# libmir/mir-optim

Hardware: AMD Instinct MI355X
Metric: LM iterations/sec (higher is better)
Workload: dtype f64

## Files before the change

mir_optim_amd/csrc/jtj_fdp.h:

```cpp
#pragma once

#include "jtj_kernel.h"

namespace mirlsq {

constexpr int kJtjFdpThreads = 8 * kWave;

template <int NCB, bool FD = true> struct JtjFdpCfg {
    static constexpr int N = 16 * NCB;
    static constexpr int RP = !FD ? 8 : ((N % 64 == 0) ? 8 : 4);
    static constexpr int RS = 4 * RP;
    static constexpr int GPS = RS / 4;
    static constexpr int NI = FD ? RP * NCB / 4 : RP * NCB / 8;
    static constexpr int SLOT_DOUBLES = RS * N + RS;
    static constexpr int LDS_BYTES = 2 * SLOT_DOUBLES * 8;
    static constexpr int THREADS = 8 * kWave;
};

typedef double fdp_v2d __attribute__((ext_vector_type(2)));

template <int NCB>
__device__ __forceinline__ void fdp_producer(const JtjArgs<double>& a, double* smem, int lane, int w, size_t s0, size_t S)
{
    using C = JtjFdpCfg<NCB>;
// ... 84 lines not shown
        pad[i] = 2 * jp >= nr;
        pcol[i] = pad[i] ? 0 : jp;
    }
    double inv0[DIFF ? NI : 1], inv1[DIFF ? NI : 1];
    if constexpr (DIFF) {
#pragma unroll
        for (int i = 0; i < NI; ++i) {
            const double t0 = a.twh[2 * pcol[i]], t1 = a.twh[2 * pcol[i] + 1];
            inv0[i] = t0 == 0 ? 0.0 : 1.0 / t0;
            inv1[i] = t1 == 0 ? 0.0 : 1.0 / t1;
        }
    }

    fdp_v2d b[2][NI];
    double yb[2] = {0, 0};
    auto issue = [&](size_t s, auto B) {
        constexpr int bb = decltype(B)::value;
        const size_t sc = s < S ? s : S - 1;
        const size_t row0 = (s0 + sc) * C::RS + C::RP * (size_t)w;
#pragma unroll
        for (int i = 0; i < NI; ++i) {
            size_t row = row0 + prow[i];
            row = row < m ? row : m - 1;
            if constexpr (DIFF) b[bb][i] = __builtin_nontemporal_load(&Jp[row * hr + pcol[i]]);
            else b[bb][i] = Jp[row * hr + pcol[i]];
        }
        size_t yr = row0 + (lane & (C::RP - 1));
        yr = yr < m ? yr : m - 1;
        yb[bb] = a.y[yr];
    };
    auto convert = [&](size_t s, auto B) {
        constexpr int bb = decltype(B)::value;
        double* slot = smem + (s & 1) * C::SLOT_DOUBLES;
        const size_t row0 = (s0 + s) * C::RS + C::RP * (size_t)w;
#pragma unroll
        for (int i = 0; i < NI; ++i) {
            fdp_v2d v = b[bb][i];
            if constexpr (DIFF) {
                v.x = inv0[i] == 0 ? 0.0 : v.x * inv0[i];
                v.y = inv1[i] == 0 ? 0.0 : v.y * inv1[i];
            }
            if (pad[i] || row0 + prow[i] >= m) v = fdp_v2d{0.0, 0.0};
            *reinterpret_cast<fdp_v2d*>(slot + w * C::RP * n + 2 * (64 * i + lane)) = v;
        }
        if (lane < C::RP) slot[C::RS * n + C::RP * w + lane] = (row0 + lane < m) ? yb[bb] : 0.0;
    };

    if (S > 0) {
        issue(0, IntC<0>{});
        issue(1, IntC<1>{});
        for (size_t t = 0; t < S; t += 2) {
            static_for<2>([&](auto U) {
                constexpr int u = decltype(U)::value;
                if (t + u < S) {
                    convert(t + u, U);
                    issue(t + u + 2, U);
                    asm volatile("s_waitcnt lgkmcnt(0)" ::: "memory");
                    __builtin_amdgcn_s_barrier();
                }
            });
        }
    }
}

template <int NCB, bool DIFF = false>
__device__ __forceinline__ void fdp_producer_plain_flat(const JtjArgs<double>& a, double* smem, int lane, int w, size_t s0, size_t S)
{
    using C = JtjFdpCfg<NCB, false>;
    constexpr int n = C::N;
    constexpr int NI = C::NI;
    const size_t m = a.m;
    const int nr = a.n;
    double* invt = smem + 2 * C::SLOT_DOUBLES;
    if constexpr (DIFF) {
        for (int c = lane; c < nr; c += kWave) { const double t = a.twh[c]; invt[c] = t == 0 ? 0.0 : 1.0 / t; }
    }
    const size_t rowb = s0 * C::RS < m ? s0 * C::RS : m;
    const size_t left = (m - rowb) * (size_t)nr * sizeof(double);
    const __amdgpu_buffer_rsrc_t rsrc = __builtin_amdgcn_make_buffer_rsrc(
        const_cast<double*>(a.J + rowb * (size_t)nr), 0, (int)(left < 0xffffffffull ? left : 0xffffffffull), 0x00020000);

    __amdgpu_buffer_rsrc_t rout = rsrc;
    if constexpr (DIFF) {
        if (a.Jout) rout = __builtin_amdgcn_make_buffer_rsrc(a.Jout + rowb * (size_t)nr, 0, (int)(left < 0xffffffffull ? left : 0xffffffffull), 0x00020000);
    }
    int off0[NI], off1[NI];
#pragma unroll
    for (int i = 0; i < NI; ++i) {
        const int e0 = 2 * (64 * i + lane), e1 = e0 + 1;
        off0[i] = e0 < C::RP * nr ? (e0 / nr) * n + e0 % nr : -1;
        off1[i] = e1 < C::RP * nr ? (e1 / nr) * n + e1 % nr : -1;
    }
    for (int e = lane; e < C::RP * (n - nr); e += kWave) {
        const int r = e / (n - nr), c = nr + e % (n - nr);
        smem[w * C::RP * n + r * n + c] = 0.0;
        smem[C::SLOT_DOUBLES + w * C::RP * n + r * n + c] = 0.0;
    }
    asm volatile("s_waitcnt lgkmcnt(0)" ::: "memory");

    typedef unsigned int fdp_u4 __attribute__((ext_vector_type(4)));
    fdp_u4 b[2][NI];
    double yb[2] = {0, 0};
    auto issue = [&](size_t s, auto B) {
        constexpr int bb = decltype(B)::value;
        const size_t sc = s < S ? s : S - 1;
        const size_t row0 = (s0 + sc) * C::RS + C::RP * (size_t)w;
        const unsigned base = (unsigned)((row0 - rowb) * (size_t)nr * sizeof(double));
#pragma unroll
        for (int i = 0; i < NI; ++i)
            b[bb][i] = __builtin_amdgcn_raw_buffer_load_b128(rsrc, (int)(base + 16u * (unsigned)(64 * i + lane)), 0, DIFF ? 2 : 0);
        size_t yr = row0 + (lane & (C::RP - 1));
        yr = yr < m ? yr : m - 1;
        yb[bb] = a.y[yr];
    };
    auto convert = [&](size_t s, auto B) {
        constexpr int bb = decltype(B)::value;
        double* slot = smem + (s & 1) * C::SLOT_DOUBLES + w * C::RP * n;
        const size_t row0 = (s0 + s) * C::RS + C::RP * (size_t)w;
        const unsigned base = (unsigned)((row0 - rowb) * (size_t)nr * sizeof(double));
#pragma unroll
        for (int i = 0; i < NI; ++i) {
            double v0 = __hiloint2double((int)b[bb][i].y, (int)b[bb][i].x), v1 = __hiloint2double((int)b[bb][i].w, (int)b[bb][i].z);
            if constexpr (DIFF) {
                const double i0 = invt[off0[i] >= 0 ? off0[i] % n : 0], i1 = invt[off1[i] >= 0 ? off1[i] % n : 0];
                v0 = i0 == 0 ? 0.0 : v0 * i0;
                v1 = i1 == 0 ? 0.0 : v1 * i1;
                if (a.Jout && off0[i] >= 0) {
                    const fdp_u4 o = {(unsigned)__double2loint(v0), (unsigned)__double2hiint(v0), (unsigned)__double2loint(v1), (unsigned)__double2hiint(v1)};
                    __builtin_amdgcn_raw_buffer_store_b128(o, rout, (int)(base + 16u * (unsigned)(64 * i + lane)), 0, 2);
                }
            }
            if (off0[i] >= 0) slot[off0[i]] = v0;
            if (off1[i] >= 0) slot[off1[i]] = v1;
        }
        if (lane < C::RP) smem[(s & 1) * C::SLOT_DOUBLES + C::RS * n + C::RP * w + lane] = (row0 + lane < m) ? yb[bb] : 0.0;
    };
    if (S > 0) {
        issue(0, IntC<0>{});
        issue(1, IntC<1>{});
        for (size_t t = 0; t < S; t += 2) {
            static_for<2>([&](auto U) {
                constexpr int u = decltype(U)::value;
                if (t + u < S) {
                    convert(t + u, U);
                    issue(t + u + 2, U);
                    asm volatile("s_waitcnt lgkmcnt(0)" ::: "memory");
                    __builtin_amdgcn_s_barrier();
                }
            });
        }
    }
}

template <int NCB, int ROLE, bool FD = true, bool DIFF = false, bool PRODUCER_WRITES_J = false>
__device__ __forceinline__ void fdp_consumer(const JtjArgs<double>& a, const double* smem, int lane, size_t s0, size_t S)
{
    using T = double;
    using Acc = typename Mma<T>::Acc;
    using C = JtjFdpCfg<NCB, FD>;
    constexpr int NACC = jtj_nacc<NCB>();
    constexpr int n = C::N;
    const int q = lane >> 4, p = lane & 15;
    const size_t m = a.m;

    Acc acc[NACC];
#pragma unroll
    for (int i = 0; i < NACC; ++i) acc[i] = Acc{0, 0, 0, 0};
    T jy[NCB];
#pragma unroll
    for (int c = 0; c < NCB; ++c) jy[c] = 0;

    for (size_t s = 0; s < S; ++s) {
        __builtin_amdgcn_s_barrier();
        const T* slot = smem + (s & 1) * C::SLOT_DOUBLES;
        const size_t row0 = (s0 + s) * C::RS;
        struct Grp { T v[NCB]; T y; };
        auto read = [&](int gi, Grp& g) {
#pragma unroll
            for (int c = 0; c < NCB; ++c) g.v[c] = slot[(4 * gi + q) * n + 16 * c + p];
            g.y = 0;
            if constexpr (ROLE == 0) g.y = slot[C::RS * n + 4 * gi + q];
        };
        auto side = [&](int gi, const Grp& g) {
            if constexpr ((FD || DIFF) && ROLE >= 2 && !PRODUCER_WRITES_J) {
                const size_t row = row0 + 4 * gi + q;
                if (row < m && a.Jout) {
                    T* wp = a.Jout + row * (size_t)a.n;
#pragma unroll
                    for (int c = 0; c < NCB; ++c)
                        if (c % 2 == ROLE - 2) { if (16 * c + p < a.n) __builtin_nontemporal_store(g.v[c], &wp[16 * c + p]); }
                }
            }
            if constexpr (ROLE == 0) {
#pragma unroll
                for (int c = 0; c < NCB; ++c) jy[c] += g.v[c] * g.y;
            }
        };
        auto mfmas = [&](const Grp& g) {
#pragma unroll
            for (int I = 0; I < NCB; ++I)
#pragma unroll
                for (int Jb2 = 0; Jb2 <= I; ++Jb2)
                    if (jtj_owns<NCB, 4, ROLE>(I * (I + 1) / 2 + Jb2))
                        acc[I * (I + 1) / 2 + Jb2] = Mma<T>::mma(g.v[I], g.v[Jb2], acc[I * (I + 1) / 2 + Jb2]);
        };
        Grp ga, gb;
        read(0, ga);
        side(0, ga);
#pragma unroll
        for (int gi = 0; gi < C::GPS; gi += 2) {
            if (gi + 1 < C::GPS) read(gi + 1, gb);
            mfmas(ga);
            if (gi + 1 < C::GPS) {
                side(gi + 1, gb);
                if (gi + 2 < C::GPS) read(gi + 2, ga);
                mfmas(gb);
                if (gi + 2 < C::GPS) side(gi + 2, ga);
            }
        }
    }

    T* dst = a.slabs + (size_t)blockIdx.x * jtj_slab_len<NCB>();
#pragma unroll
    for (int i = 0; i < NACC; ++i)
        if (jtj_owns<NCB, 4, ROLE>(i)) {
#pragma unroll
            for (int r = 0; r < 4; ++r) dst[(i * 4 + r) * kWave + lane] = acc[i][r];
        }
    if constexpr (ROLE == 0) {
#pragma unroll
        for (int c = 0; c < NCB; ++c) {
            jy[c] += wave_shfl_xor(jy[c], 16);
            jy[c] += wave_shfl_xor(jy[c], 32);
            dst[(NACC * 4 + c) * kWave + lane] = jy[c];
        }
    }
}

template <int NCB, bool FD = true, bool DIFF = false, bool ELEM = false>
__global__ __launch_bounds__(kJtjFdpThreads) __attribute__((amdgpu_waves_per_eu(4, 4))) void k_jtj_fdp(JtjArgs<double> a)
{
    static_assert(!(FD && DIFF), "DIFF uses the plain stage layout");
    static_assert(!(FD && ELEM), "the pair panel's rows always start on 16-byte boundaries");
    using C = JtjFdpCfg<NCB, FD>;
    extern __shared__ __attribute__((aligned(16))) unsigned char fdp_smem[];
    double* smem = reinterpret_cast<double*>(fdp_smem);
    const int lane = threadIdx.x & 63;
    const int wave = __builtin_amdgcn_readfirstlane(threadIdx.x >> 6);

    const size_t Stot = (a.m + C::RS - 1) / C::RS;
    const size_t per = (Stot + gridDim.x - 1) / gridDim.x;
    const size_t s0 = (size_t)blockIdx.x * per < Stot ? (size_t)blockIdx.x * per : Stot;
    const size_t s1 = s0 + per < Stot ? s0 + per : Stot;
    const size_t S = s1 - s0;

    constexpr bool PW = DIFF && ELEM;
    if (wave == 0) fdp_consumer<NCB, 0, FD, DIFF, PW>(a, smem, lane, s0, S);
    else if (wave == 1) fdp_consumer<NCB, 1, FD, DIFF, PW>(a, smem, lane, s0, S);
    else if (wave == 2) fdp_consumer<NCB, 2, FD, DIFF, PW>(a, smem, lane, s0, S);
    else if (wave == 3) fdp_consumer<NCB, 3, FD, DIFF, PW>(a, smem, lane, s0, S);
    else if constexpr (FD) fdp_producer<NCB>(a, smem, lane, wave - 4, s0, S);
    else if constexpr (ELEM) fdp_producer_plain_flat<NCB, DIFF>(a, smem, lane, wave - 4, s0, S);
    else fdp_producer_plain<NCB, DIFF>(a, smem, lane, wave - 4, s0, S);
}

}
```

mir_optim_amd/csrc/workloads_gemm.hip:

```cpp
#include "workloads_gemm.h"
#include "workloads_device.h"

namespace {

template <int NK>
__global__ __launch_bounds__(1024) void k_tanh_linear_batched(const double* __restrict__ A, const double* __restrict__ b,
                                                               const double* __restrict__ X, double* __restrict__ Y,
                                                               size_t m, int n, int P)
{
    using Acc = __attribute__((ext_vector_type(4))) double;
    constexpr int NPAD = 4 * NK;
    constexpr int PITCH = NPAD + 2;
    __shared__ __attribute__((aligned(16))) double tile[2][16 * PITCH];
    const int tid = threadIdx.x, lane = tid & 63, wave = tid >> 6;
    const int fr = lane & 15, fq = lane >> 4;

    for (int idx = tid; idx < 2 * 16 * PITCH; idx += 1024) (&tile[0][0])[idx] = 0.0;
    __syncthreads();

    const int ppr = n / 2;
    const bool has_piece = tid < 16 * ppr;
    const int prow = has_piece ? tid / ppr : 0, pcol = has_piece ? tid % ppr : 0;
    const size_t ntiles = (m + 15) / 16;

    for (int pbase = 0; pbase < P; pbase += 256) {
        const int pl = pbase + wave * 16 + fr;
        const bool pok = pl < P;
        const bool wave_active = pbase + wave * 16 < P;
        double xf[NK];
#pragma unroll
        for (int s = 0; s < NK; ++s) {
            const int col = 4 * s + fq;
            xf[s] = (pok && col < n) ? X[(size_t)pl * n + col] : 0.0;
        }
        double2 stage = make_double2(0.0, 0.0);
        auto gload = [&](size_t t) {
            const size_t row = t * 16 + prow;
            if (has_piece && row < m) stage = *reinterpret_cast<const double2*>(A + row * (size_t)n + 2 * pcol);
            else stage = make_double2(0.0, 0.0);
        };
        auto lstore = [&](int buf) {
            if (has_piece) *reinterpret_cast<double2*>(&tile[buf][prow * PITCH + 2 * pcol]) = stage;
        };
        size_t t = blockIdx.x;
        if (t < ntiles) { gload(t); lstore(0); }
        if (t + gridDim.x < ntiles) gload(t + gridDim.x);
        __syncthreads();
        int buf = 0;
        Acc prev = {0.0, 0.0, 0.0, 0.0};
        size_t tprev = ntiles;
        auto epilogue = [&](const Acc& acc, size_t tt) {
#pragma unroll
            for (int r = 0; r < 4; ++r) {
                const size_t row = tt * 16 + fq + 4 * r;
                if (pok && tt < ntiles && row < m) Y[(size_t)pl * m + row] = dtanh(acc[r]) - b[row];
            }
        };
        for (; t < ntiles; t += gridDim.x) {
            if (wave_active) {
                Acc acc = {0.0, 0.0, 0.0, 0.0};
                const double* tp = &tile[buf][fr * PITCH + fq];
#pragma unroll
                for (int s = 0; s < NK; ++s) acc = __builtin_amdgcn_mfma_f64_16x16x4f64(tp[4 * s], xf[s], acc, 0, 0, 0);
                epilogue(prev, tprev);
                prev = acc;
                tprev = t;
            }
            if (t + gridDim.x < ntiles) lstore(buf ^ 1);
            if (t + 2 * (size_t)gridDim.x < ntiles) gload(t + 2 * (size_t)gridDim.x);
            __syncthreads();
            buf ^= 1;
        }
        if (wave_active) epilogue(prev, tprev);
        __syncthreads();
    }
}


typedef __attribute__((address_space(3))) void* wl_lds_ptr;
typedef const __attribute__((address_space(1))) void* wl_gbl_ptr;

__device__ __forceinline__ constexpr int tlb_rho(int i) { return ((i >> 2) >> 1) * 8 + 2 * (i & 3) + ((i >> 2) & 1); }
__device__ __forceinline__ constexpr int tlb_sigma(int i) { return (i + 12) & 15; }

template <int NK> struct TlbCfg {
    static constexpr int N = 4 * NK;
    static constexpr int PPR = N / 2;
    static constexpr int TILES = NK <= 32 ? 2 : 1;
    static constexpr bool SELF = NK > 32;
    static constexpr int COMPUTE_WAVES = 8, LOADER_WAVES = SELF ? 0 : 2;
    static constexpr int CHUNK = 16 * COMPUTE_WAVES;
    static constexpr int ROWS = 16 * TILES;
    static constexpr int STAGE_BYTES = ROWS * N * 8;
    static constexpr int IPS = STAGE_BYTES / 1024;
    static constexpr int NS = 4, D = 2, NSB = 8;
    static constexpr int B_OFF = NS * STAGE_BYTES;
    static constexpr int LDS_BYTES = B_OFF + NSB * 256;
    static constexpr int THREADS = 64 * (COMPUTE_WAVES + LOADER_WAVES);
    static constexpr bool FORK = NK == 32;
    static constexpr int NPRE = NK / 2 - 1;
    static constexpr int PRE_STAGE = TILES * NPRE * 16 * 8;
    static constexpr int PRE_OFF = LDS_BYTES;
    static constexpr int VOTE_OFF = PRE_OFF + 2 * PRE_STAGE;
    static constexpr int FORK_LDS_BYTES = VOTE_OFF + 16;
    static constexpr int BASE_OFF = FORK_LDS_BYTES;
    static constexpr int BASE_LDS_BYTES = BASE_OFF + N * 8;
};

__device__ __forceinline__ int tlb_lane_now()
{
    int l;
    asm volatile("v_mbcnt_lo_u32_b32 %0, -1, 0\n\tv_mbcnt_hi_u32_b32 %0, -1, %0" : "=v"(l));
    return l;
}
template <int NK>
__device__ __forceinline__ void tlb_base_rows(const unsigned char* slot, const unsigned char* bslot, const unsigned char* smem,
                                              double* __restrict__ ybase, size_t row0, size_t m, int wave)
{
    using C = TlbCfg<NK>;
    static_assert(C::N == 128 && C::ROWS == 32 && C::COMPUTE_WAVES == 8, "four rows a wave, four column pairs a lane");
    const int lane = tlb_lane_now();
    const int q = lane >> 4, p = lane & 15;
    const int R = 4 * wave + q;
    const unsigned char* rp = slot + R * C::N * 8 + (p ^ tlb_sigma(R & 15)) * 16;
    const unsigned char* xp = smem + C::BASE_OFF + p * 16;
    double s = 0.0;
#pragma unroll
    for (int h = 0; h < 2; ++h) {
        double v0[2], v1[2], x0[2], x1[2];
#pragma unroll
        for (int c = 0; c < 2; ++c) {
            const double2 a = *reinterpret_cast<const double2*>(rp + (2 * h + c) * 256);
            const double2 x = *reinterpret_cast<const double2*>(xp + (2 * h + c) * 256);
            v0[c] = a.x; v1[c] = a.y;
            x0[c] = x.x; x1[c] = x.y;
        }
        s = tanh_linear_row_sum<double, 2>(v0, v1, x0, x1, s);
        __builtin_amdgcn_sched_barrier(0);
    }
    s = sum16(s);
    const double t = dtanh(s);
    const int lr = (R & 16) + tlb_rho(R & 15);
    const double bv = *reinterpret_cast<const double*>(bslot + lr * 8);
    const int rows = m - row0 < (size_t)C::ROWS ? (int)(m - row0) : C::ROWS;
    if (p == 0 && lr < rows) (ybase + row0)[lr] = t - bv;
}

__host__ __device__ constexpr int tlb_fork_group(int w, int which)
{
    constexpr int T[8][2] = {{2, 15}, {3, 14}, {0, 13}, {1, 12}, {6, 11}, {7, 10}, {4, 9}, {5, 8}};
    return T[w][which];
}
constexpr bool tlb_fork_groups_ok()
{
    int owners[16] = {};
    for (int w = 0; w < 8; ++w) {
        if (tlb_fork_group(w, 0) >= tlb_fork_group(w, 1)) return false;
        for (int which = 0; which < 2; ++which) {
            const int g = tlb_fork_group(w, which);
            if (g < 0 || g > 15) return false;
            ++owners[g];
        }
    }
    for (int g = 0; g < 16; ++g)
        if (owners[g] != 1) return false;
    return true;
}
static_assert(tlb_fork_groups_ok(), "every 16-point group 0..15 belongs to exactly one compute wave");

template <int NK, int LOADER>
__device__ __forceinline__ void tlb_issue(const double* __restrict__ A, const double* __restrict__ b, size_t m,
                                          unsigned char* smem, int lane, size_t S, size_t f)
{
    using C = TlbCfg<NK>;
    constexpr int MYI = C::IPS / 2;
    const unsigned char* Ab = reinterpret_cast<const unsigned char*>(A);
    const unsigned char* bb = reinterpret_cast<const unsigned char*>(b);
    const size_t stage = blockIdx.x + (f % S) * (size_t)gridDim.x;
    const size_t row0 = stage * C::ROWS;
    unsigned char* slot = smem + (f % C::NS) * C::STAGE_BYTES;
#pragma unroll
    for (int k = 0; k < MYI; ++k) {
        const int ins = LOADER + 2 * k;
        const int g = ins * 64 + lane;
        const int R = g / C::PPR, sp = g % C::PPR;
        size_t row = row0 + (R & 16) + tlb_rho(R & 15);
        row = row < m ? row : m - 1;
        const int piece = sp ^ tlb_sigma(R & 15);
        __builtin_amdgcn_global_load_lds((wl_gbl_ptr)(Ab + (row * C::N + 2 * piece) * 8),
                                         (wl_lds_ptr)(slot + ins * 1024), 16, 0, 2 );
    }
    if constexpr (LOADER == 1) {
        size_t row = row0 + (lane >> 1);
        row = row < m ? row : m - 1;
        __builtin_amdgcn_global_load_lds((wl_gbl_ptr)(bb + row * 8 + (lane & 1) * 4),
                                         (wl_lds_ptr)(smem + C::B_OFF + (f % C::NSB) * 256), 4, 0, 0);
    }
}

template <int NK, int LOADER>
__device__ __forceinline__ void tlb_loader(const double* __restrict__ A, const double* __restrict__ b, size_t m,
                                           unsigned char* smem, int lane, size_t S, size_t F)
{
    using C = TlbCfg<NK>;
    constexpr int OPS = C::IPS / 2 + (LOADER == 1 ? 1 : 0);
    auto issue = [&](size_t f) { tlb_issue<NK, LOADER>(A, b, m, smem, lane, S, f); };
    const size_t pre = F < (size_t)C::D ? F : (size_t)C::D;
    for (size_t f = 0; f < pre; ++f) issue(f);
    for (size_t f = 0; f < F; ++f) {
        if (f + C::D < F) {
            issue(f + C::D);
            asm volatile("s_waitcnt vmcnt(%0)" ::"n"(C::D * OPS) : "memory");
        } else {
            asm volatile("s_waitcnt vmcnt(0)" ::: "memory");
        }
        __builtin_amdgcn_s_barrier();
    }
}

template <int NK, bool ALIGNED, int GROUP, bool RM = false, bool DIFF = false>
__device__ __forceinline__ void tlb_compute(const double* __restrict__ A, const double* __restrict__ b,
                                            const double* __restrict__ X, double* __restrict__ Y, size_t m, int P,
                                            unsigned char* smem, int lane, int wave, size_t S, int nchunks)
{
    using C = TlbCfg<NK>;
    using Acc = __attribute__((ext_vector_type(4))) double;
    const int fr = lane & 15, fq = lane >> 4;
    const int v = fq ^ tlb_sigma(fr);
    int laddr[4];
#pragma unroll
    for (int k = 0; k < 4; ++k) laddr[k] = fr * C::N * 8 + ((4 * k) ^ v) * 16;

    constexpr int MYI = C::SELF ? C::IPS / C::COMPUTE_WAVES : 1;
    [[maybe_unused]] int roff[MYI], soff[MYI];
    [[maybe_unused]] unsigned is_next = 0, slot_next = 0, bslot_next = 0;
    [[maybe_unused]] const size_t Ftot = S * (size_t)nchunks;
    [[maybe_unused]] size_t fissued = 0;
    const unsigned char* Ab = reinterpret_cast<const unsigned char*>(A);
    const unsigned char* bb = reinterpret_cast<const unsigned char*>(b);
    if constexpr (C::SELF) {
#pragma unroll
        for (int k = 0; k < MYI; ++k) {
            const int g = (wave + C::COMPUTE_WAVES * k) * 64 + lane;
            const int R = g / C::PPR, sp = g % C::PPR;
            roff[k] = (R & 16) + tlb_rho(R & 15);
            soff[k] = 2 * (sp ^ tlb_sigma(R & 15)) * 8;
        }
    }
    auto issue = [&]() {
        const size_t row0 = (blockIdx.x + (size_t)is_next * gridDim.x) * C::ROWS;
        unsigned char* slot = smem + slot_next * C::STAGE_BYTES;
#pragma unroll
        for (int k = 0; k < MYI; ++k) {
            size_t row = row0 + roff[k];
            row = row < m ? row : m - 1;
            __builtin_amdgcn_global_load_lds((wl_gbl_ptr)(Ab + row * (C::N * 8) + soff[k]),
                                             (wl_lds_ptr)(slot + (wave + C::COMPUTE_WAVES * k) * 1024), 16, 0, 2 );
        }
        if (wave == 0) {
            size_t row = row0 + (lane >> 1);
            row = row < m ? row : m - 1;
            __builtin_amdgcn_global_load_lds((wl_gbl_ptr)(bb + row * 8 + (lane & 1) * 4),
                                             (wl_lds_ptr)(smem + C::B_OFF + bslot_next * 256), 4, 0, 0);
        }
        is_next = is_next + 1 == (unsigned)S ? 0 : is_next + 1;
        slot_next = (slot_next + 1) % C::NS;
        bslot_next = (bslot_next + 1) % C::NSB;
        ++fissued;
    };
    auto advance = [&]() {
        if constexpr (C::SELF) {
            if (fissued < Ftot) {
                issue();
                if (wave == 0) asm volatile("s_waitcnt vmcnt(%0)" ::"n"(C::D * (MYI + 1)) : "memory");
                else asm volatile("s_waitcnt vmcnt(%0)" ::"n"(C::D * MYI) : "memory");
            } else {
                asm volatile("s_waitcnt vmcnt(0)" ::: "memory");
            }
        }
    };
    if constexpr (C::SELF) {
        for (int d = 0; d < C::D && fissued < Ftot; ++d) issue();
        advance();
    }

    size_t f = 0;
    for (int ch = 0; ch < nchunks; ++ch) {
        const bool wave_active = ch * C::CHUNK + wave * 16 < P;
        if (!wave_active) {
            for (size_t s = 0; s < S; ++s) {
                __builtin_amdgcn_s_barrier();
                ++f;
                if (f < Ftot) advance();
            }
            continue;
        }
        int pl = ch * C::CHUNK + wave * 16 + fr;
        pl = pl < P ? pl : P - 1;
        double xf[NK];
#pragma unroll
        for (int s = 0; s < NK; ++s) xf[s] = X[(size_t)pl * C::N + 8 * (s >> 1) + 2 * fq + (s & 1)];
        double* yp = DIFF ? Y + (pl >> 1) : (RM ? Y + pl : Y + (size_t)pl * m);
        const size_t ldr = DIFF ? (size_t)(P >> 1) : (RM ? (size_t)P : 1);
// ... 137 lines not shown
        dp[c] = D + j;
    }
    constexpr size_t ldr = N;

    auto mfma_stage = [&](size_t st, auto cc, Acc& acc0, Acc& acc1) {
        constexpr int c = decltype(cc)::value;
        const unsigned char* slot = smem + (st % C::NS) * C::STAGE_BYTES;
        acc0 = Acc{0, 0, 0, 0};
        acc1 = Acc{0, 0, 0, 0};
        auto xop = [&](int s) { return (hit[c] && sstar[c] == s) ? xs[c] : xb[s]; };
        if constexpr (C::TILES == 2) {
#pragma unroll
            for (int j = 0; j < NK / 2; ++j) {
                const int off = laddr[j & 3] + (j >> 2) * 256;
                const double2 a0 = *reinterpret_cast<const double2*>(slot + off);
                const double2 a1 = *reinterpret_cast<const double2*>(slot + off + 16 * N * 8);
                const double x0 = xop(2 * j), x1 = xop(2 * j + 1);
                acc0 = __builtin_amdgcn_mfma_f64_16x16x4f64(a0.x, x0, acc0, 0, 0, 0);
                acc1 = __builtin_amdgcn_mfma_f64_16x16x4f64(a1.x, x0, acc1, 0, 0, 0);
                acc0 = __builtin_amdgcn_mfma_f64_16x16x4f64(a0.y, x1, acc0, 0, 0, 0);
                acc1 = __builtin_amdgcn_mfma_f64_16x16x4f64(a1.y, x1, acc1, 0, 0, 0);
            }
        } else {
#pragma unroll
            for (int j = 0; j < NK / 2; j += 2) {
                const double2 a0 = *reinterpret_cast<const double2*>(slot + laddr[j & 3] + (j >> 2) * 256);
                const double2 a1 = *reinterpret_cast<const double2*>(slot + laddr[(j + 1) & 3] + ((j + 1) >> 2) * 256);
                acc0 = __builtin_amdgcn_mfma_f64_16x16x4f64(a0.x, xop(2 * j), acc0, 0, 0, 0);
                acc1 = __builtin_amdgcn_mfma_f64_16x16x4f64(a1.x, xop(2 * j + 2), acc1, 0, 0, 0);
                acc0 = __builtin_amdgcn_mfma_f64_16x16x4f64(a0.y, xop(2 * j + 1), acc0, 0, 0, 0);
                acc1 = __builtin_amdgcn_mfma_f64_16x16x4f64(a1.y, xop(2 * j + 3), acc1, 0, 0, 0);
            }
            acc0 += acc1;
        }
    };
    auto epilogue_tile = [&](const Acc& acc, size_t row0, const unsigned char* bslot, double* yp, bool full) {
        const double2 b0 = *reinterpret_cast<const double2*>(bslot + 16 * fq);
        const double2 b1 = *reinterpret_cast<const double2*>(bslot + 64 + 16 * fq);
        const double y0 = dtanh(acc[0]) - b0.x, y1 = dtanh(acc[1]) - b0.y;
        const double y2 = dtanh(acc[2]) - b1.x, y3 = dtanh(acc[3]) - b1.y;
        const double d0 = y0 - lane_pair_swap(y0), d1 = y1 - lane_pair_swap(y1);
        const double d2 = y2 - lane_pair_swap(y2), d3 = y3 - lane_pair_swap(y3);
        const size_t ra = row0 + 2 * fq, rb = row0 + 8 + 2 * fq;
        if ((fr & 1) == 0) {
            if (full || ra < m) yp[ra * ldr] = d0;
            if (full || ra + 1 < m) yp[(ra + 1) * ldr] = d1;
            if (full || rb < m) yp[rb * ldr] = d2;
            if (full || rb + 1 < m) yp[(rb + 1) * ldr] = d3;
        }
    };
    auto epilogue = [&](const Acc& e0, const Acc& e1, size_t st, auto cc) {
        constexpr int c = decltype(cc)::value;
        const size_t row0 = (blockIdx.x + st * (size_t)gridDim.x) * C::ROWS;
        const unsigned char* bs = smem + C::B_OFF + (st % C::NSB) * 256;
        const bool full = st + 1 < S;
        epilogue_tile(e0, row0, bs, dp[c], full);
        __builtin_amdgcn_sched_barrier(0);
        if constexpr (C::TILES == 2) {
            epilogue_tile(e1, row0 + 16, bs + 128, dp[c], full);
            __builtin_amdgcn_sched_barrier(0);
        }
    };
    Acc acc0, acc1;
    if constexpr (GROUP == 0) {
        for (size_t st = 0; st < S; ++st) {
            __builtin_amdgcn_s_barrier();
            wl_static_for<NCH>([&](auto cc) {
                if (act[decltype(cc)::value]) {
                    mfma_stage(st, cc, acc0, acc1);
                    epilogue(acc0, acc1, st, cc);
                }
            });
        }
    } else {
        for (size_t st = 0; st < S; ++st) {
            wl_static_for<NCH>([&](auto cc) {
                constexpr int c = decltype(cc)::value;
                if constexpr (c == 0) {
                    __builtin_amdgcn_s_barrier();
                    if (st > 0) {
                        wl_static_for<NCH>([&](auto pp) {
                            constexpr int pc = decltype(pp)::value;
                            constexpr bool last = pc == NCH - 1;
                            if (act[pc] && (last || !act[pc + (last ? 0 : 1)])) epilogue(acc0, acc1, st - 1, pp);
                        });
                    }
                    if (act[0]) mfma_stage(st, cc, acc0, acc1);
                } else {
                    if (act[c]) {
                        epilogue(acc0, acc1, st, std::integral_constant<int, c - 1>{});
                        mfma_stage(st, cc, acc0, acc1);
                    }
                }
            });
        }
        if (S > 0) {
            wl_static_for<NCH>([&](auto pp) {
                constexpr int pc = decltype(pp)::value;
                constexpr bool last = pc == NCH - 1;
                if (act[pc] && (last || !act[pc + (last ? 0 : 1)])) epilogue(acc0, acc1, S - 1, pp);
            });
        }
    }
}


template <int NK>
__device__ __forceinline__ bool tlb_fork_vote(const double* __restrict__ X, unsigned char* smem, int lane, int wave)
{
    using C = TlbCfg<NK>;
    constexpr int N = C::N, P = 2 * N;
    volatile int* vote = reinterpret_cast<volatile int*>(smem + C::VOTE_OFF);
    if (threadIdx.x == 0) *vote = 0;
    __syncthreads();
    if (wave < C::COMPUTE_WAVES) {
        const int fr = lane & 15, fq = lane >> 4;
        const int s0 = 2 * tlb_fork_group(wave, 0), s1 = 2 * tlb_fork_group(wave, 1);
        const unsigned long long* xr = reinterpret_cast<const unsigned long long*>(X);
        const unsigned long long* x0 = xr + (size_t)(8 * s0 + fr) * N;
        const unsigned long long* x1 = xr + (size_t)(8 * s1 + fr) * N;
        bool bad = false;
#pragma unroll
        for (int s = 0; s < NK - 2; ++s) {
            const int k = 8 * (s >> 1) + 2 * fq + (s & 1);
            const unsigned long long xb = xr[(size_t)((2 * k + 2) % P) * N + k];
            const unsigned long long a = x0[k], c = x1[k];
            bad |= (s < s0) & (a != xb);
            bad |= (s < s1) & (c != xb);
        }
        if (bad) *vote = 1;
    }
    __syncthreads();
    return *vote == 0;
}

template <int NK, int LOADER>
__device__ __forceinline__ void tlb_fork_loader(const double* __restrict__ A, const double* __restrict__ b,
                                                const double* __restrict__ X, size_t m, unsigned char* smem, int lane, size_t S)
{
    using C = TlbCfg<NK>;
    constexpr int N = C::N, P = 2 * N;
    constexpr int OPS = C::IPS / 2 + (LOADER == 1 ? 1 : 0);
    const int fr = lane & 15, fq = lane >> 4;
    const int v = fq ^ tlb_sigma(fr);
    int laddr[4];
#pragma unroll
    for (int k = 0; k < 4; ++k) laddr[k] = LOADER * 16 * N * 8 + fr * N * 8 + ((4 * k) ^ v) * 16;
    double xb[2 * C::NPRE];
#pragma unroll
    for (int s = 0; s < 2 * C::NPRE; ++s) {
        const int k = 8 * (s >> 1) + 2 * fq + (s & 1);
        xb[s] = X[(size_t)((2 * k + 2) % P) * N + k];
    }
    auto issue = [&](size_t f) { tlb_issue<NK, LOADER>(A, b, m, smem, lane, S, f); };
    for (size_t f = 0; f < S && f < (size_t)C::D; ++f) issue(f);
    for (size_t f = 0; f < S; ++f) {
        if (f + 1 < S) asm volatile("s_waitcnt vmcnt(%0)" ::"n"(OPS) : "memory");
        else asm volatile("s_waitcnt vmcnt(0)" ::: "memory");
        __builtin_amdgcn_s_barrier();
        asm volatile("" ::: "memory");
        if (f + C::D < S) issue(f + C::D);
        const unsigned char* slot = smem + (f % C::NS) * C::STAGE_BYTES;
        double* pre = reinterpret_cast<double*>(smem + C::PRE_OFF + (f & 1) * C::PRE_STAGE) + LOADER * C::NPRE * 16 + 4 * fq + (fr >> 2);
        double acc = 0.0;
#pragma unroll
        for (int j = 0; j < C::NPRE; ++j) {
            const double2 a = *reinterpret_cast<const double2*>(slot + laddr[j & 3] + (j >> 2) * 256);
            acc = __builtin_amdgcn_mfma_f64_4x4x4f64(a.x, xb[2 * j], acc, 0, 0, 0);
            acc = __builtin_amdgcn_mfma_f64_4x4x4f64(a.y, xb[2 * j + 1], acc, 0, 0, 0);
            if ((fr & 3) == 0) pre[16 * j] = acc;
        }
        asm volatile("s_waitcnt lgkmcnt(0)" ::: "memory");
    }
    __builtin_amdgcn_s_barrier();
}

template <int NK, int W, bool BASE = false>
__device__ __forceinline__ void tlb_fork_compute(const double* __restrict__ X, double* __restrict__ D, size_t m,
                                                 unsigned char* smem, int lane, size_t S)
{
    using C = TlbCfg<NK>;
    using Acc = __attribute__((ext_vector_type(4))) double;
    constexpr int N = C::N;
    constexpr int GA = tlb_fork_group(W, 0), GC = tlb_fork_group(W, 1);
    constexpr int SA = 2 * GA, SC = 2 * GC;
    constexpr int GROUP = W < C::COMPUTE_WAVES / 2 ? 0 : 1;
    const int fr = lane & 15, fq = lane >> 4;
    const int v = fq ^ tlb_sigma(fr);
    int laddr[4];
#pragma unroll
    for (int k = 0; k < 4; ++k) laddr[k] = fr * N * 8 + ((4 * k) ^ v) * 16;
    const int pa = 16 * GA + fr, pc = 16 * GC + fr;
    double xa[NK - SA], xc[NK - SC];
#pragma unroll
    for (int s = SA; s < NK; ++s) xa[s - SA] = X[(size_t)pa * N + 8 * (s >> 1) + 2 * fq + (s & 1)];
#pragma unroll
    for (int s = SC; s < NK; ++s) xc[s - SC] = X[(size_t)pc * N + 8 * (s >> 1) + 2 * fq + (s & 1)];
    constexpr size_t ldr = N;
    constexpr int DC = 8 * (GC - GA);
    const unsigned voff = (unsigned)(((pa >> 1) + 2 * fq * ldr) * 8);
    unsigned char* sb = reinterpret_cast<unsigned char*>(D + (size_t)blockIdx.x * C::ROWS * ldr);
    const size_t stage_step = (size_t)gridDim.x * C::ROWS * ldr * 8;

    auto mfma_stage = [&](size_t f, Acc (&acc)[4]) {
        const unsigned char* slot = smem + (f % C::NS) * C::STAGE_BYTES;
        const double* pre = reinterpret_cast<const double*>(smem + C::PRE_OFF + (f & 1) * C::PRE_STAGE) + 4 * fq;
        auto prefix = [&](int t, int s) {
            if (s == 0) return Acc{0.0, 0.0, 0.0, 0.0};
            const double* p = pre + (t * C::NPRE + s / 2 - 1) * 16;
            const double2 lo = *reinterpret_cast<const double2*>(p), hi = *reinterpret_cast<const double2*>(p + 2);
            return Acc{lo.x, lo.y, hi.x, hi.y};
        };
        acc[0] = prefix(0, SA);
        acc[1] = prefix(1, SA);
        acc[2] = prefix(0, SC);
        acc[3] = prefix(1, SC);
        wl_static_for<NK / 2 - GA>([&](auto jj) {
            constexpr int j = GA + decltype(jj)::value;
            const int off = laddr[j & 3] + (j >> 2) * 256;
            const double2 a0 = *reinterpret_cast<const double2*>(slot + off);
            const double2 a1 = *reinterpret_cast<const double2*>(slot + off + 16 * N * 8);
            acc[0] = __builtin_amdgcn_mfma_f64_16x16x4f64(a0.x, xa[2 * j - SA], acc[0], 0, 0, 0);
            acc[1] = __builtin_amdgcn_mfma_f64_16x16x4f64(a1.x, xa[2 * j - SA], acc[1], 0, 0, 0);
            if constexpr (j >= GC) {
                acc[2] = __builtin_amdgcn_mfma_f64_16x16x4f64(a0.x, xc[2 * j - SC], acc[2], 0, 0, 0);
                acc[3] = __builtin_amdgcn_mfma_f64_16x16x4f64(a1.x, xc[2 * j - SC], acc[3], 0, 0, 0);
            }
            acc[0] = __builtin_amdgcn_mfma_f64_16x16x4f64(a0.y, xa[2 * j + 1 - SA], acc[0], 0, 0, 0);
            acc[1] = __builtin_amdgcn_mfma_f64_16x16x4f64(a1.y, xa[2 * j + 1 - SA], acc[1], 0, 0, 0);
            if constexpr (j >= GC) {
                acc[2] = __builtin_amdgcn_mfma_f64_16x16x4f64(a0.y, xc[2 * j + 1 - SC], acc[2], 0, 0, 0);
                acc[3] = __builtin_amdgcn_mfma_f64_16x16x4f64(a1.y, xc[2 * j + 1 - SC], acc[3], 0, 0, 0);
            }
        });
    };
    auto epilogue_tile = [&](const Acc& acc, unsigned char* yb, size_t ra, const unsigned char* bslot, auto full_tag) {
        constexpr bool FULL = decltype(full_tag)::value;
        const double2 b0 = *reinterpret_cast<const double2*>(bslot + 16 * fq);
        const double2 b1 = *reinterpret_cast<const double2*>(bslot + 64 + 16 * fq);
        const double y0 = dtanh(acc[0]) - b0.x, y1 = dtanh(acc[1]) - b0.y;
        const double y2 = dtanh(acc[2]) - b1.x, y3 = dtanh(acc[3]) - b1.y;
        const double d0 = y0 - lane_pair_swap(y0), d1 = y1 - lane_pair_swap(y1);
        const double d2 = y2 - lane_pair_swap(y2), d3 = y3 - lane_pair_swap(y3);
        double* const yp = reinterpret_cast<double*>(yb + voff);
        if ((fr & 1) == 0) {
            if (FULL || ra < m) yp[0] = d0;
            if (FULL || ra + 1 < m) yp[ldr] = d1;
            if (FULL || ra + 8 < m) yp[8 * ldr] = d2;
            if (FULL || ra + 9 < m) yp[9 * ldr] = d3;
        }
    };
    auto epilogue = [&](const Acc (&acc)[4], size_t f, auto full_tag) {
        const size_t ra = (blockIdx.x + f * (size_t)gridDim.x) * C::ROWS + 2 * fq;
        const unsigned char* bs = smem + C::B_OFF + (f % C::NSB) * 256;
        epilogue_tile(acc[0], sb, ra, bs, full_tag);
        __builtin_amdgcn_sched_barrier(0);
        epilogue_tile(acc[1], sb + 16 * ldr * 8, ra + 16, bs + 128, full_tag);
        __builtin_amdgcn_sched_barrier(0);
        epilogue_tile(acc[2], sb + DC * 8, ra, bs, full_tag);
        __builtin_amdgcn_sched_barrier(0);
        epilogue_tile(acc[3], sb + (DC + 16 * ldr) * 8, ra + 16, bs + 128, full_tag);
        __builtin_amdgcn_sched_barrier(0);
        sb += stage_step;
    };
    auto barrier = [] {
        asm volatile("" ::: "memory");
        __builtin_amdgcn_s_barrier();
        asm volatile("" ::: "memory");
    };
    constexpr int BASE_SHARES = !BASE || W == 2 || W == 3 ? 0 : W >= 6 ? 2 : 1;
    [[maybe_unused]] auto base_rows = [&](size_t f) {
        wl_static_for<BASE_SHARES>([&](auto hh) {
            tlb_base_rows<NK>(smem + (f % C::NS) * C::STAGE_BYTES, smem + C::B_OFF + (f % C::NSB) * 256, smem, D + m * ldr,
                              (blockIdx.x + f * (size_t)gridDim.x) * C::ROWS, m, W - 4 * decltype(hh)::value);
            __builtin_amdgcn_sched_barrier(0);
        });
    };
    Acc acc[4];
    barrier();
    if constexpr (GROUP == 0) {
        for (size_t f = 0; f < S; ++f) {
            barrier();
            base_rows(f);
            mfma_stage(f, acc);
            if (f + 1 < S) epilogue(acc, f, std::true_type{});
            else epilogue(acc, f, std::false_type{});
        }
    } else {
        barrier();
        base_rows(0);
        mfma_stage(0, acc);
        for (size_t f = 1; f < S; ++f) {
            barrier();
            epilogue(acc, f - 1, std::true_type{});
            base_rows(f);
            mfma_stage(f, acc);
        }
        epilogue(acc, S - 1, std::false_type{});
    }
}

template <int NK>
__device__ __forceinline__ void tlb_base_sweep(const double* __restrict__ A, const double* __restrict__ b, const double* __restrict__ x,
                                               double* __restrict__ ybase, size_t m, int wave, size_t S)
{
    using C = TlbCfg<NK>;
    static_assert(C::N == 128, "four column pairs a lane");
    const int lane = tlb_lane_now();
    const int q = lane >> 4, p = lane & 15;
    double x0[4], x1[4];
#pragma unroll
    for (int c = 0; c < 4; ++c) {
        const double2 t = *reinterpret_cast<const double2*>(x + 32 * c + 2 * p);
        x0[c] = t.x; x1[c] = t.y;
    }
    for (size_t k = wave; k < S; k += C::THREADS / 64) {
        const size_t row0 = (blockIdx.x + k * (size_t)gridDim.x) * C::ROWS;
        for (int g = 0; g < C::ROWS / 4; ++g) {
            const size_t row = row0 + 4 * g + q, rc = row < m ? row : m - 1;
            double v0[4], v1[4];
#pragma unroll
            for (int c = 0; c < 4; ++c) {
                const double2 t = *reinterpret_cast<const double2*>(A + rc * C::N + 32 * c + 2 * p);
                v0[c] = t.x; v1[c] = t.y;
            }
            const double s = sum16(tanh_linear_row_sum<double, 4>(v0, v1, x0, x1));
            const double t = dtanh(s);
            if (p == 0 && row < m) ybase[row] = t - b[rc];
        }
    }
}

template <int NK, bool RM = false, bool DIFF = false, bool BASE = false>
__global__ __launch_bounds__(TlbCfg<NK>::THREADS) void k_tanh_linear_batched_dma(const double* __restrict__ A,
                                                                                  const double* __restrict__ b,
                                                                                  const double* __restrict__ X,
                                                                                  double* __restrict__ Y, size_t m, int P,
                                                                                  int mode)
{
    using C = TlbCfg<NK>;
    extern __shared__ __attribute__((aligned(16))) unsigned char tlb_smem[];
    const int lane = threadIdx.x & 63;
    const int wave = __builtin_amdgcn_readfirstlane(threadIdx.x >> 6);
    const size_t Stot = (m + C::ROWS - 1) / C::ROWS;
    const size_t S = blockIdx.x < Stot ? (Stot - blockIdx.x + gridDim.x - 1) / gridDim.x : 0;
    const int nchunks = (P + C::CHUNK - 1) / C::CHUNK;
    const bool once = DIFF && mode == 1 && NK <= 32 && P == 2 * C::N;
    const size_t F = once ? S : S * (size_t)nchunks;
    if (S == 0) return;
    if constexpr (BASE) {
        static_assert(DIFF && C::FORK, "the extra point rides on the n = 128 difference panel");
        if (threadIdx.x < C::N) reinterpret_cast<double*>(tlb_smem + C::BASE_OFF)[threadIdx.x] = X[(size_t)P * C::N + threadIdx.x];
        __syncthreads();
    }
    if constexpr (DIFF && C::FORK) {
        if (mode == 2 && P == 2 * C::N && tlb_fork_vote<NK>(X, tlb_smem, lane, wave)) {
            if (wave == C::COMPUTE_WAVES) tlb_fork_loader<NK, 0>(A, b, X, m, tlb_smem, lane, S);
            else if (wave == C::COMPUTE_WAVES + 1) tlb_fork_loader<NK, 1>(A, b, X, m, tlb_smem, lane, S);
            else wl_static_for<C::COMPUTE_WAVES>([&](auto ww) {
                if (wave == decltype(ww)::value) tlb_fork_compute<NK, decltype(ww)::value, BASE>(X, Y, m, tlb_smem, lane, S);
            });
            return;
        }
    }
    if (!C::SELF && wave == C::COMPUTE_WAVES) tlb_loader<NK, 0>(A, b, m, tlb_smem, lane, S, F);
    else if (!C::SELF && wave == C::COMPUTE_WAVES + 1) tlb_loader<NK, 1>(A, b, m, tlb_smem, lane, S, F);
    else if (DIFF && once) {
        if constexpr (DIFF) {
            if (wave < 4) tlb_compute_once<NK, 0>(X, Y, m, tlb_smem, lane, wave, S);
            else tlb_compute_once<NK, 1>(X, Y, m, tlb_smem, lane, wave, S);
        }
    } else {
        if constexpr (RM) {
            if (wave < 4) tlb_compute<NK, false, 0, true, DIFF>(A, b, X, Y, m, P, tlb_smem, lane, wave, S, nchunks);
            else tlb_compute<NK, false, 1, true, DIFF>(A, b, X, Y, m, P, tlb_smem, lane, wave, S, nchunks);
        } else {
            const bool aligned = ((m & 1) == 0) && ((reinterpret_cast<uintptr_t>(Y) & 15) == 0);
            if (wave < 4) {
                if (aligned) tlb_compute<NK, true, 0>(A, b, X, Y, m, P, tlb_smem, lane, wave, S, nchunks);
                else tlb_compute<NK, false, 0>(A, b, X, Y, m, P, tlb_smem, lane, wave, S, nchunks);
            } else {
                if (aligned) tlb_compute<NK, true, 1>(A, b, X, Y, m, P, tlb_smem, lane, wave, S, nchunks);
                else tlb_compute<NK, false, 1>(A, b, X, Y, m, P, tlb_smem, lane, wave, S, nchunks);
            }
        }
    }
    if constexpr (BASE) tlb_base_sweep<NK>(A, b, X + (size_t)P * C::N, Y + m * (size_t)C::N, m, wave, S);
}

template <int NK, bool RM = false, bool DIFF = false, bool BASE = false>
bool launch_tlb_dma(const double* A, const double* b, const double* X, double* Y, size_t m, int P, hipStream_t s, int mode = 0)
{
    using C = TlbCfg<NK>;
    constexpr int lds = BASE ? C::BASE_LDS_BYTES : DIFF && C::FORK ? C::FORK_LDS_BYTES : C::LDS_BYTES;
    static bool attr_ok = [] {
        return hipFuncSetAttribute(reinterpret_cast<const void*>(k_tanh_linear_batched_dma<NK, RM, DIFF, BASE>),
                                   hipFuncAttributeMaxDynamicSharedMemorySize, lds) == hipSuccess;
    }();
    if (!attr_ok) return false;
    const size_t Stot = (m + C::ROWS - 1) / C::ROWS;
    const unsigned grid = (unsigned)(Stot < 256 ? Stot : 256);
    hipLaunchKernelGGL((k_tanh_linear_batched_dma<NK, RM, DIFF, BASE>), dim3(grid), dim3(C::THREADS), lds, s, A, b, X, Y, m, P, mode);
    return true;
}

__global__ __launch_bounds__(256) void k_tanh_linear_batched_rm_generic(const double* __restrict__ A, const double* __restrict__ b,
                                                                        const double* __restrict__ X, double* __restrict__ Y,
                                                                        size_t m, int n, int P)
{
    const size_t total = m * (size_t)P;
    for (size_t e = (size_t)blockIdx.x * blockDim.x + threadIdx.x; e < total; e += (size_t)gridDim.x * blockDim.x) {
        const size_t i = e / P;
        const int k = (int)(e % P);
        const double* a = A + i * (size_t)n;
        const double* x = X + (size_t)k * n;
        double s0 = 0;
// ... 165 lines not shown
```

Baseline: 1184.

## Balance J stores and Jᵀy across consumer roles with buffer stores and read-ahead ring

Reassigns the per-column side work (J writeback and the Jᵀy accumulation) from fixed roles (ROLE 0 for jy, roles 2/3 for stores) to a compile-time load-balanced owner per column, interleaved right after that column's first MFMA in each role. Global stores switch to raw buffer stores with a per-stage resource descriptor whose range check replaces the per-row bounds branch. The two-group ping-pong is replaced by a ring with configurable read-ahead depth and sched barriers to keep LDS reads ahead of the MFMAs. The aim is to even out work across the four consumer waves and hide LDS latency, at the cost of more registers for the deeper ring and rigid scheduling.

```diff
diff --git a/mir_optim_amd/csrc/jtj_fdp.h b/mir_optim_amd/csrc/jtj_fdp.h
--- a/mir_optim_amd/csrc/jtj_fdp.h
+++ b/mir_optim_amd/csrc/jtj_fdp.h
@@ -260,6 +260,41 @@
     }
 }
 
+template <int NCB> __host__ __device__ constexpr bool fdp_role_reads(int role, int c)
+{
+    constexpr int per = (jtj_nacc<NCB>() + 3) / 4;
+    for (int I = 0; I < NCB; ++I)
+        for (int Jb = 0; Jb <= I; ++Jb)
+            if ((I == c || Jb == c) && (I * (I + 1) / 2 + Jb) / per == role) return true;
+    return false;
+}
+template <int NCB> __host__ __device__ constexpr int fdp_side_owner(int c)
+{
+    constexpr int per = (jtj_nacc<NCB>() + 3) / 4;
+    int load[4] = {0, 0, 0, 0};
+    for (int r = 0; r < 4; ++r) {
+        const int left = jtj_nacc<NCB>() - r * per;
+        load[r] = left < 0 ? 0 : (left < per ? left : per);
+    }
+    int owner = 0;
+    for (int cc = NCB - 1; cc >= c; --cc) {
+        owner = -1;
+        for (int r = 0; r < 4; ++r)
+            if (fdp_role_reads<NCB>(r, cc) && (owner < 0 || load[r] < load[owner])) owner = r;
+        ++load[owner];
+    }
+    return owner;
+}
+template <int NCB, int ROLE> __host__ __device__ constexpr int fdp_first_use(int c)
+{
+    for (int I = 0; I < NCB; ++I)
+        for (int Jb = 0; Jb <= I; ++Jb)
+            if ((I == c || Jb == c) && jtj_owns<NCB, 4, ROLE>(I * (I + 1) / 2 + Jb)) return I * (I + 1) / 2 + Jb;
+    return -1;
+}
+
+typedef unsigned int fdp_u2 __attribute__((ext_vector_type(2)));
+
 template <int NCB, int ROLE, bool FD = true, bool DIFF = false, bool PRODUCER_WRITES_J = false>
 __device__ __forceinline__ void fdp_consumer(const JtjArgs<double>& a, const double* smem, int lane, size_t s0, size_t S)
 {
@@ -268,6 +303,8 @@
     using C = JtjFdpCfg<NCB, FD>;
     constexpr int NACC = jtj_nacc<NCB>();
     constexpr int n = C::N;
+    constexpr bool STORES = (FD || DIFF) && !PRODUCER_WRITES_J;
+    constexpr unsigned kNoColumn = 0xC0000000u;
     const int q = lane >> 4, p = lane & 15;
     const size_t m = a.m;
 
@@ -275,57 +312,60 @@
 #pragma unroll
     for (int i = 0; i < NACC; ++i) acc[i] = Acc{0, 0, 0, 0};
     T jy[NCB];
-#pragma unroll
-    for (int c = 0; c < NCB; ++c) jy[c] = 0;
+    unsigned coff[NCB];
+#pragma unroll
+    for (int c = 0; c < NCB; ++c) {
+        jy[c] = 0;
+        coff[c] = 16 * c + p < a.n ? (unsigned)(q * a.n + 16 * c + p) * 8u : kNoColumn;
+    }
+    const unsigned gstep = 32u * (unsigned)a.n;
 
     for (size_t s = 0; s < S; ++s) {
+        const size_t row0 = (s0 + s) * C::RS;
+        const size_t rows = row0 < m ? (m - row0 < (size_t)C::RS ? m - row0 : (size_t)C::RS) : 0;
+        T* const jbase = a.Jout ? a.Jout + (row0 < m ? row0 : m) * (size_t)a.n : nullptr;
+        const __amdgpu_buffer_rsrc_t jrs = __builtin_amdgcn_make_buffer_rsrc(jbase, 0, jbase ? (int)(rows * (size_t)a.n * sizeof(T)) : 0, 0x00020000);
         __builtin_amdgcn_s_barrier();
         const T* slot = smem + (s & 1) * C::SLOT_DOUBLES;
-        const size_t row0 = (s0 + s) * C::RS;
         struct Grp { T v[NCB]; T y; };
         auto read = [&](int gi, Grp& g) {
 #pragma unroll
             for (int c = 0; c < NCB; ++c) g.v[c] = slot[(4 * gi + q) * n + 16 * c + p];
-            g.y = 0;
-            if constexpr (ROLE == 0) g.y = slot[C::RS * n + 4 * gi + q];
+            g.y = slot[C::RS * n + 4 * gi + q];
         };
-        auto side = [&](int gi, const Grp& g) {
-            if constexpr ((FD || DIFF) && ROLE >= 2 && !PRODUCER_WRITES_J) {
-                const size_t row = row0 + 4 * gi + q;
-                if (row < m && a.Jout) {
-                    T* wp = a.Jout + row * (size_t)a.n;
-#pragma unroll
-                    for (int c = 0; c < NCB; ++c)
-                        if (c % 2 == ROLE - 2) { if (16 * c + p < a.n) __builtin_nontemporal_store(g.v[c], &wp[16 * c + p]); }
+        auto side = [&](unsigned goff, int c, const Grp& g) {
+            if constexpr (STORES)
+                __builtin_amdgcn_raw_buffer_store_b64(fdp_u2{(unsigned)__double2loint(g.v[c]), (unsigned)__double2hiint(g.v[c])}, jrs,
+                                                      (int)(coff[c] + goff), 0, 2);
+            jy[c] = __builtin_fma(g.v[c], g.y, jy[c]);
+        };
+        auto work = [&](int gi, const Grp& g) {
+            unsigned goff = (unsigned)gi * gstep;
+            if constexpr (STORES) asm volatile("" : "+s"(goff));
+#pragma unroll
+            for (int I = 0; I < NCB; ++I)
+#pragma unroll
+                for (int Jb2 = 0; Jb2 <= I; ++Jb2) {
+                    const int b = I * (I + 1) / 2 + Jb2;
+                    if (jtj_owns<NCB, 4, ROLE>(b)) {
+                        acc[b] = Mma<T>::mma(g.v[I], g.v[Jb2], acc[b]);
+#pragma unroll
+                        for (int c = 0; c < NCB; ++c)
+                            if ((c == I || c == Jb2) && fdp_side_owner<NCB>(c) == ROLE && fdp_first_use<NCB, ROLE>(c) == b) side(goff, c, g);
+                    }
                 }
-            }
-            if constexpr (ROLE == 0) {
-#pragma unroll
-                for (int c = 0; c < NCB; ++c) jy[c] += g.v[c] * g.y;
-            }
         };
-        auto mfmas = [&](const Grp& g) {
-#pragma unroll
-            for (int I = 0; I < NCB; ++I)
-#pragma unroll
-                for (int Jb2 = 0; Jb2 <= I; ++Jb2)
-                    if (jtj_owns<NCB, 4, ROLE>(I * (I + 1) / 2 + Jb2))
-                        acc[I * (I + 1) / 2 + Jb2] = Mma<T>::mma(g.v[I], g.v[Jb2], acc[I * (I + 1) / 2 + Jb2]);
-        };
-        Grp ga, gb;
-        read(0, ga);
-        side(0, ga);
-#pragma unroll
-        for (int gi = 0; gi < C::GPS; gi += 2) {
-            if (gi + 1 < C::GPS) read(gi + 1, gb);
-            mfmas(ga);
-            if (gi + 1 < C::GPS) {
-                side(gi + 1, gb);
-                if (gi + 2 < C::GPS) read(gi + 2, ga);
-                mfmas(gb);
-                if (gi + 2 < C::GPS) side(gi + 2, ga);
-            }
-        }
+        constexpr int AHEAD = NCB >= 7 ? 1 : (NCB >= 5 ? 2 : 3), RING = AHEAD + 1;
+        static_assert(AHEAD < C::GPS, "the prologue reads AHEAD groups of the stage");
+        Grp gr[RING];
+        static_for<AHEAD>([&](auto U) { read(decltype(U)::value, gr[decltype(U)::value]); });
+        static_for<C::GPS>([&](auto G) {
+            constexpr int gi = decltype(G)::value;
+            if constexpr (gi + AHEAD < C::GPS) read(gi + AHEAD, gr[(gi + AHEAD) % RING]);
+            __builtin_amdgcn_sched_barrier(0);
+            work(gi, gr[gi % RING]);
+            __builtin_amdgcn_sched_barrier(0);
+        });
     }
 
     T* dst = a.slabs + (size_t)blockIdx.x * jtj_slab_len<NCB>();
@@ -335,14 +375,13 @@
 #pragma unroll
             for (int r = 0; r < 4; ++r) dst[(i * 4 + r) * kWave + lane] = acc[i][r];
         }
-    if constexpr (ROLE == 0) {
-#pragma unroll
-        for (int c = 0; c < NCB; ++c) {
+#pragma unroll
+    for (int c = 0; c < NCB; ++c)
+        if (fdp_side_owner<NCB>(c) == ROLE) {
             jy[c] += wave_shfl_xor(jy[c], 16);
             jy[c] += wave_shfl_xor(jy[c], 32);
             dst[(NACC * 4 + c) * kWave + lane] = jy[c];
         }
-    }
 }
 
 template <int NCB, bool FD = true, bool DIFF = false, bool ELEM = false>
```

Measured after the change: 1189 (median of 2 runs). About the same (+0.5%).

## Inline loader DMA issue with precomputed offsets and scalarize epilogue store bases

Applied to the files above, without the earlier changes.

Replaces the generic tlb_issue call in the loader waves with an inlined issue path. It precomputes per-lane swizzled A offsets and advances uniform base pointers, so each stage issues one global_load_lds per LDS row with minimal address arithmetic. A bounds-clamped path is kept only for the last stage. The compute epilogue forces its store base pointers into scalar registers via readfirstlane and uses compile-time column offsets with global address-space stores, cutting VGPR address math. The compute-wave group pairing table is also reshuffled, which changes the per-wave load balance and LDS access pattern.

```diff
diff --git a/mir_optim_amd/csrc/workloads_gemm.hip b/mir_optim_amd/csrc/workloads_gemm.hip
--- a/mir_optim_amd/csrc/workloads_gemm.hip
+++ b/mir_optim_amd/csrc/workloads_gemm.hip
@@ -148,7 +148,7 @@
 
 __host__ __device__ constexpr int tlb_fork_group(int w, int which)
 {
-    constexpr int T[8][2] = {{2, 15}, {3, 14}, {0, 13}, {1, 12}, {6, 11}, {7, 10}, {4, 9}, {5, 8}};
+    constexpr int T[8][2] = {{1, 15}, {5, 11}, {0, 14}, {4, 10}, {3, 13}, {7, 9}, {2, 12}, {6, 8}};
     return T[w][which];
 }
 constexpr bool tlb_fork_groups_ok()
@@ -592,7 +592,54 @@
         const int k = 8 * (s >> 1) + 2 * fq + (s & 1);
         xb[s] = X[(size_t)((2 * k + 2) % P) * N + k];
     }
-    auto issue = [&](size_t f) { tlb_issue<NK, LOADER>(A, b, m, smem, lane, S, f); };
+    constexpr int MYI = C::IPS / 2;
+    static_assert(C::PPR == 64 && C::STAGE_BYTES == C::ROWS * N * 8, "one DMA instruction per LDS row");
+    unsigned aoff[MYI];
+#pragma unroll
+    for (int k = 0; k < MYI; ++k) {
+        const int R = LOADER + 2 * k;
+        aoff[k] = (unsigned)(((R & 16) + tlb_rho(R & 15)) * N * 8 + (lane ^ tlb_sigma(R & 15)) * 16);
+        asm volatile("" : "+v"(aoff[k]));
+    }
+    unsigned boff = (unsigned)lane * 4;
+    asm volatile("" : "+v"(boff));
+    const unsigned char* anext = reinterpret_cast<const unsigned char*>(A) + (size_t)blockIdx.x * C::STAGE_BYTES;
+    const unsigned char* bnext = reinterpret_cast<const unsigned char*>(b) + (size_t)blockIdx.x * (C::ROWS * 8);
+    const size_t astep = (size_t)gridDim.x * C::STAGE_BYTES, bstep = (size_t)gridDim.x * (C::ROWS * 8);
+    auto issue = [&](size_t f) {
+        unsigned char* slot = smem + (f % C::NS) * C::STAGE_BYTES;
+        unsigned char* bslot = smem + C::B_OFF + (f % C::NSB) * 256;
+        if (f + 1 < S) {
+#pragma unroll
+            for (int k = 0; k < MYI; ++k) {
+                asm volatile("" : "+v"(aoff[k]));
+                __builtin_amdgcn_global_load_lds((wl_gbl_ptr)(anext + aoff[k]), (wl_lds_ptr)(slot + (LOADER + 2 * k) * 1024), 16, 0, 2 );
+            }
+            if constexpr (LOADER == 1) {
+                asm volatile("" : "+v"(boff));
+                __builtin_amdgcn_global_load_lds((wl_gbl_ptr)(bnext + boff), (wl_lds_ptr)bslot, 4, 0, 0);
+            }
+        } else {
+            const unsigned char* Ab = reinterpret_cast<const unsigned char*>(A);
+            const size_t row0 = (blockIdx.x + f * (size_t)gridDim.x) * C::ROWS;
+#pragma unroll
+            for (int k = 0; k < MYI; ++k) {
+                const int R = LOADER + 2 * k;
+                size_t row = row0 + (R & 16) + tlb_rho(R & 15);
+                row = row < m ? row : m - 1;
+                const unsigned piece = (unsigned)((lane ^ tlb_sigma(R & 15)) * 16);
+                __builtin_amdgcn_global_load_lds((wl_gbl_ptr)(Ab + row * (N * 8) + piece), (wl_lds_ptr)(slot + R * 1024), 16, 0, 2 );
+            }
+            if constexpr (LOADER == 1) {
+                size_t row = row0 + (lane >> 1);
+                row = row < m ? row : m - 1;
+                __builtin_amdgcn_global_load_lds((wl_gbl_ptr)(reinterpret_cast<const unsigned char*>(b) + row * 8 + (lane & 1) * 4),
+                                                 (wl_lds_ptr)bslot, 4, 0, 0);
+            }
+        }
+        anext += astep;
+        bnext += bstep;
+    };
     for (size_t f = 0; f < S && f < (size_t)C::D; ++f) issue(f);
     for (size_t f = 0; f < S; ++f) {
         if (f + 1 < S) asm volatile("s_waitcnt vmcnt(%0)" ::"n"(OPS) : "memory");
@@ -615,6 +662,13 @@
     __builtin_amdgcn_s_barrier();
 }
 
+__device__ __forceinline__ unsigned char* tlb_uniform_ptr(unsigned char* p)
+{
+    const unsigned long long u = reinterpret_cast<unsigned long long>(p);
+    const unsigned lo = __builtin_amdgcn_readfirstlane((unsigned)u), hi = __builtin_amdgcn_readfirstlane((unsigned)(u >> 32));
+    return reinterpret_cast<unsigned char*>(((unsigned long long)hi << 32) | lo);
+}
+
 template <int NK, int W, bool BASE = false>
 __device__ __forceinline__ void tlb_fork_compute(const double* __restrict__ X, double* __restrict__ D, size_t m,
                                                  unsigned char* smem, int lane, size_t S)
@@ -638,8 +692,9 @@
     for (int s = SC; s < NK; ++s) xc[s - SC] = X[(size_t)pc * N + 8 * (s >> 1) + 2 * fq + (s & 1)];
     constexpr size_t ldr = N;
     constexpr int DC = 8 * (GC - GA);
-    const unsigned voff = (unsigned)(((pa >> 1) + 2 * fq * ldr) * 8);
-    unsigned char* sb = reinterpret_cast<unsigned char*>(D + (size_t)blockIdx.x * C::ROWS * ldr);
+    unsigned voff = (unsigned)(((pa >> 1) + 2 * fq * ldr) * 8);
+    asm volatile("" : "+v"(voff));
+    unsigned char* sb = tlb_uniform_ptr(reinterpret_cast<unsigned char*>(D + (size_t)blockIdx.x * C::ROWS * ldr));
     const size_t stage_step = (size_t)gridDim.x * C::ROWS * ldr * 8;
 
     auto mfma_stage = [&](size_t f, Acc (&acc)[4]) {
@@ -674,34 +729,44 @@
             }
         });
     };
-    auto epilogue_tile = [&](const Acc& acc, unsigned char* yb, size_t ra, const unsigned char* bslot, auto full_tag) {
+    auto epilogue_tile = [&](const Acc& acc, unsigned char* yb, auto col_tag, size_t ra, const unsigned char* bslot, auto full_tag) {
         constexpr bool FULL = decltype(full_tag)::value;
+        constexpr int COL = decltype(col_tag)::value;
+        unsigned char* yr0 = yb;
+        unsigned char* yr8 = yb + 8 * ldr * 8;
+        asm volatile("" : "+v"(voff));
+        yr0 = tlb_uniform_ptr(yr0);
+        yr8 = tlb_uniform_ptr(yr8);
         const double2 b0 = *reinterpret_cast<const double2*>(bslot + 16 * fq);
         const double2 b1 = *reinterpret_cast<const double2*>(bslot + 64 + 16 * fq);
         const double y0 = dtanh(acc[0]) - b0.x, y1 = dtanh(acc[1]) - b0.y;
         const double y2 = dtanh(acc[2]) - b1.x, y3 = dtanh(acc[3]) - b1.y;
         const double d0 = y0 - lane_pair_swap(y0), d1 = y1 - lane_pair_swap(y1);
         const double d2 = y2 - lane_pair_swap(y2), d3 = y3 - lane_pair_swap(y3);
-        double* const yp = reinterpret_cast<double*>(yb + voff);
+        typedef __attribute__((address_space(1))) double* gbl_double_ptr;
+        const gbl_double_ptr p0 = (gbl_double_ptr)(yr0 + voff + COL);
+        const gbl_double_ptr p8 = (gbl_double_ptr)(yr8 + voff + COL);
         if ((fr & 1) == 0) {
-            if (FULL || ra < m) yp[0] = d0;
-            if (FULL || ra + 1 < m) yp[ldr] = d1;
-            if (FULL || ra + 8 < m) yp[8 * ldr] = d2;
-            if (FULL || ra + 9 < m) yp[9 * ldr] = d3;
+            if (FULL || ra < m) p0[0] = d0;
+            if (FULL || ra + 1 < m) p0[ldr] = d1;
+            if (FULL || ra + 8 < m) p8[0] = d2;
+            if (FULL || ra + 9 < m) p8[ldr] = d3;
         }
     };
     auto epilogue = [&](const Acc (&acc)[4], size_t f, auto full_tag) {
         const size_t ra = (blockIdx.x + f * (size_t)gridDim.x) * C::ROWS + 2 * fq;
         const unsigned char* bs = smem + C::B_OFF + (f % C::NSB) * 256;
-        epilogue_tile(acc[0], sb, ra, bs, full_tag);
+        constexpr std::integral_constant<int, 0> col_a{};
+        constexpr std::integral_constant<int, DC * 8> col_c{};
+        epilogue_tile(acc[0], sb, col_a, ra, bs, full_tag);
         __builtin_amdgcn_sched_barrier(0);
-        epilogue_tile(acc[1], sb + 16 * ldr * 8, ra + 16, bs + 128, full_tag);
+        epilogue_tile(acc[1], sb + 16 * ldr * 8, col_a, ra + 16, bs + 128, full_tag);
         __builtin_amdgcn_sched_barrier(0);
-        epilogue_tile(acc[2], sb + DC * 8, ra, bs, full_tag);
+        epilogue_tile(acc[2], sb, col_c, ra, bs, full_tag);
         __builtin_amdgcn_sched_barrier(0);
-        epilogue_tile(acc[3], sb + (DC + 16 * ldr) * 8, ra + 16, bs + 128, full_tag);
+        epilogue_tile(acc[3], sb + 16 * ldr * 8, col_c, ra + 16, bs + 128, full_tag);
         __builtin_amdgcn_sched_barrier(0);
-        sb += stage_step;
+        sb = tlb_uniform_ptr(sb + stage_step);
     };
     auto barrier = [] {
         asm volatile("" ::: "memory");
```

Result: faster. 1181 before, 1200 after, median of 6 (+1.5%).
